# hellosunking/Microcket

Measured on AMD Instinct MI355X. Metric: read-pairs/sec through sam2pairs+dedup (150 bp PE, hg38 names, SAM text resident in HBM), higher is better.
Workload: dtype u8; 1 GPU; C2: 100 M 150 bp PE Micro-C read pairs, hg38, one MI355X -- 100000000 synthetic 150 bp PE read pairs per GPU, hg38 chromosome names, 1 lane(s), unc mode, sam=no, seed 20260105, one step = one pass over the whole resident data set + duplicate marking of the reported pairs on (chr1,pos1,chr2,pos2,strands) + per-chromosome-pair counts; preset=C2, pairs_per_gpu=100000001, sam_bytes_per_gpu=94584442002, block_groups=2097152, blocks=48, parallelism=shard1: independent read-group shards, no data-path collective

## Files before the change

### microcket_amd/csrc/mkt_capi.cpp

```cpp
#include <hip/hip_runtime.h>
#include <stdarg.h>
#include <stdio.h>
#include <stdlib.h>
#include <string.h>
#include <algorithm>
#include <string>
#include <utility>
#include <chrono>
#include <condition_variable>
#include <deque>
#include <mutex>
#include <thread>
#include <vector>

#include "../../include/mkt.h"
#include "mkt_launch.h"

using namespace mkt;

static const size_t kMaxBlock = ((size_t)1 << 31) - 65536;

static thread_local std::string g_create_error;

struct mkt_ctx {
// ... 84 lines not shown
#define HIPCHK(c, call)                                                                            \
    do {                                                                                           \
        hipError_t e_ = (call);                                                                    \
        if (e_ != hipSuccess) return fail((c), MKT_E_HIP, "%s failed: %s", #call, hipGetErrorString(e_)); \
    } while (0)

extern "C" {

int mkt_abi_version(void) { return MKT_ABI_VERSION; }

const char* mkt_strerror(int code) {
    switch (code) {
    case MKT_OK: return "ok";
    case MKT_E_ARG: return "bad argument";
    case MKT_E_NO_DEVICE: return "no usable HIP device (this library has no CPU path)";
    case MKT_E_HIP: return "HIP runtime error";
    case MKT_E_NOMEM: return "out of memory";
    case MKT_E_CAPACITY: return "a QNAME group does not fit the block buffer";
    case MKT_E_KERNEL: return "kernel reported an internal error";
    case MKT_E_STATE: return "call order violated";
    case MKT_E_IO: return "temporary file error";
    default: return "unknown error";
    }
}
const char* mkt_last_error(const mkt_ctx* ctx) { return ctx ? ctx->err.c_str() : g_create_error.c_str(); }

int mkt_device_count(void) {
    int n = 0;
    if (hipGetDeviceCount(&n) != hipSuccess) return 0;
    return n;
}

static size_t ws_tiles_bytes(uint32_t ntiles) {
    size_t b = (size_t)ntiles * (3 * sizeof(uint64_t) + sizeof(TileLast) + sizeof(uint64_t) + sizeof(uint32_t));
    return (b + 127) & ~(size_t)127;
}
static size_t ws_fixed_bytes() { return kMaxRegions * sizeof(RegionCur) + 256 + 1024 * sizeof(uint64_t); }
static size_t ws_bytes_for(uint32_t ntiles) { return ws_tiles_bytes(ntiles) + ws_fixed_bytes() + sizeof(BlockResult); }
static int sync_all(mkt_ctx* c) {
    if (c->s_in) HIPCHK(c, hipStreamSynchronize(c->s_in));
    if (c->stream) HIPCHK(c, hipStreamSynchronize(c->stream));
    if (c->s_out) HIPCHK(c, hipStreamSynchronize(c->s_out));
    return MKT_OK;
}
static int ensure_ws(mkt_ctx* c, uint32_t ntiles) {
    size_t need = ws_bytes_for(ntiles);
    if (need <= c->ws_cap) return MKT_OK;
    need += need / 4;
    if (c->d_ws) { int rc = sync_all(c); if (rc) return rc; HIPCHK(c, hipFree(c->d_ws)); }
    c->d_ws = nullptr; c->ws_cap = 0;
    HIPCHK(c, hipMalloc((void**)&c->d_ws, need));
    c->ws_cap = need;
    return MKT_OK;
}
static int ensure_dev(mkt_ctx* c, uint8_t** p, size_t* cap, size_t need) {
    if (need <= *cap) return MKT_OK;
    if (*p) { int rc = sync_all(c); if (rc) return rc; HIPCHK(c, hipFree(*p)); }
    *p = nullptr; *cap = 0;
    need += need / 8 + 4096;
    HIPCHK(c, hipMalloc((void**)p, need));
    *cap = need;
    return MKT_OK;
}

int mkt_create(const mkt_params* p, mkt_ctx** out) {
    if (!p || !out) return fail(nullptr, MKT_E_ARG, "null argument");
    *out = nullptr;
    if (p->mode != MKT_MODE_FLASH && p->mode != MKT_MODE_UNC) return fail(nullptr, MKT_E_ARG, "mode must be MKT_MODE_FLASH or MKT_MODE_UNC");
    if (p->ref_threads < 2) return fail(nullptr, MKT_E_ARG, "ref_threads must be >= 2 (sam2pairs.cpp:36)");
    int ndev = 0;
// ... 119 lines not shown
    if (!c->d_probe) {
        if (hipMalloc((void**)&c->d_probe, sizeof(unsigned long long)) != hipSuccess) return 0;
        if (hipHostMalloc((void**)&c->h_probe, sizeof(unsigned long long), hipHostMallocDefault) != hipSuccess) return 0;
    }
    if (hipMemsetAsync(c->d_probe, 0, sizeof(unsigned long long), c->stream) != hipSuccess) return 0;
    if (launch_count_newlines(d_text, look, c->d_probe, c->stream) != hipSuccess) return 0;
    if (hipMemcpyAsync(c->h_probe, c->d_probe, sizeof(unsigned long long), hipMemcpyDeviceToHost, c->stream) != hipSuccess) return 0;
    if (hipStreamSynchronize(c->stream) != hipSuccess) return 0;
    return *c->h_probe ? (double)look / (double)*c->h_probe : (double)look;
}
static void smaller_geometry(mkt_ctx* c, const uint8_t* d_text, size_t n) {
    if (c->cfg != CFG_SMALL && d_text) {
        const double avg = probe_device_lines(c, d_text, n);
        const TileDims d = avg > 0 ? lean_dims(avg) : c->dims;
        if (d.tile < c->dims.tile) { c->dims = d; return; }
    }
    if (!shrink_dims(c)) { c->cfg = CFG_SMALL; c->dims = small_dims(); }
}

struct StreamOut { uint8_t* gp; size_t gp_cap; uint8_t* gs; size_t gs_cap; hipEvent_t k0, k1, done; };
static int enqueue_block(mkt_ctx* c, const uint8_t* d_text, size_t n, int cfg, const TileDims& dims, size_t slot, const StreamOut* so = nullptr) {
    if (((uintptr_t)d_text & 15u) != 0) return fail(c, MKT_E_ARG, "block text must be 16-byte aligned");
    if (n >= kMaxBlock) return fail(c, MKT_E_ARG, "block of %zu bytes: must be < 2 GiB - 64 KiB", n);
    const uint32_t ntiles = num_tiles((uint32_t)n, dims.tile);
    int rc = ensure_ws(c, ntiles);
    if (rc) return rc;
    if ((rc = ensure_dev(c, &c->d_pairs, &c->pairs_cap, n / 3 + 65536))) return rc;
    if (c->P.write_sam && (rc = ensure_dev(c, &c->d_sam, &c->sam_cap, n + n / 4 + 65536))) return rc;
    if (!c->d_sc && (rc = ensure_sc_list(c, 1))) return rc;
    KArgs a;
    memset(&a, 0, sizeof a);
    uint8_t* w = c->d_ws;
    a.text = d_text; a.n = (uint32_t)n; a.ntiles = ntiles; a.dims = dims; a.P = c->P;
    a.descA = (uint64_t*)w; w += (size_t)ntiles * 8;
    a.descB = (uint64_t*)w; w += (size_t)ntiles * 8;
    a.descC = (uint64_t*)w; w += (size_t)ntiles * 8;
    a.tile_last = (TileLast*)w; w += (size_t)ntiles * sizeof(TileLast);
    a.tile_groups = (uint64_t*)w; w += (size_t)ntiles * sizeof(uint64_t);
    a.defer_list = (uint32_t*)w;
    w = c->d_ws + ws_tiles_bytes(ntiles);
    a.cur = (RegionCur*)w; w += kMaxRegions * sizeof(RegionCur);
    a.ticket = (uint32_t*)w;
    a.defer_count = (uint32_t*)(w + 64);
    uint32_t* ticket2 = (uint32_t*)(w + 128);
    a.last_tile = (int*)(w + 192);
    a.scan_ticket = (uint32_t*)(w + 224);
    w += 256;
    a.scan_desc = (uint64_t*)w; w += 1024 * sizeof(uint64_t);
    if ((ntiles + finish_chunk_tiles() - 1) / finish_chunk_tiles() > 1024) return fail(c, MKT_E_ARG, "block has too many tiles for the finish scan");
    a.res = (BlockResult*)w;
    a.ordered = c->p.ordered ? 1 : 0;
    a.run = c->d_run;
    a.nregions = c->p.ordered ? 1 : kMaxRegions;
    {
        const size_t need = (size_t)a.nregions * ((n / 256 / (size_t)a.nregions) * 2 + 1024);
        if (c->sc_tmp_cap < need) {
            if (c->d_sc_tmp) { if ((rc = sync_all(c))) return rc; HIPCHK(c, hipFree(c->d_sc_tmp)); }
            c->d_sc_tmp = nullptr; c->sc_tmp_cap = 0;
            HIPCHK(c, hipMalloc((void**)&c->d_sc_tmp, need * sizeof(uint64_t)));
            c->sc_tmp_cap = need;
        }
    }
    a.pairs_rcap = (c->pairs_cap / a.nregions) & ~(uint64_t)15;
    a.sam_rcap = c->P.write_sam ? ((c->sam_cap / a.nregions) & ~(uint64_t)15) : 0;
    a.sc_rcap = c->sc_tmp_cap / a.nregions;
    a.out.pairs = c->d_pairs; a.out.pairs_cap = c->pairs_cap;
    a.out.sam = c->d_sam; a.out.sam_cap = c->P.write_sam ? c->sam_cap : 0;
    a.out.sc = c->d_sc_tmp; a.out.sc_cap = c->sc_tmp_cap;
    a.sc_list = c->d_sc; a.sc_list_cap = c->sc_cap;
    if (c->p.extensions & MKT_EXT_KEYS) {
        if (!c->d_chr) { HIPCHK(c, hipMalloc((void**)&c->d_chr, sizeof(ChrTab))); HIPCHK(c, hipMemsetAsync(c->d_chr, 0, sizeof(ChrTab), c->stream)); }
        const size_t per = (n / 64 / (size_t)a.nregions) * 2 + 4096, need = per * a.nregions;
        if (c->keys_raw_cap < need) {
            if (c->d_keys_raw) { if ((rc = sync_all(c))) return rc; HIPCHK(c, hipFree(c->d_keys_raw)); }
            c->d_keys_raw = nullptr; c->keys_raw_cap = 0;
            HIPCHK(c, hipMalloc((void**)&c->d_keys_raw, need * sizeof(KeyRec)));
            c->keys_raw_cap = need;
        }
        const double per_byte = c->key_density > 0 ? (c->key_density * 2 < 1.0 / 64 ? c->key_density * 2 : 1.0 / 64) : 1.0 / 64;
        const size_t want = (size_t)c->acc.emitted + (size_t)((double)(c->bytes_unsynced + n) * per_byte) + 65536;
        if (c->key_list_cap < want) {
            size_t ncap = c->key_list_cap ? c->key_list_cap * 2 : ((size_t)1 << 22);
            while (ncap < want) ncap *= 2;
            KeyRec* nl = nullptr;
            HIPCHK(c, hipStreamSynchronize(c->stream));
            HIPCHK(c, hipMalloc((void**)&nl, ncap * sizeof(KeyRec)));
            if (c->d_key_list) { HIPCHK(c, hipMemcpy(nl, c->d_key_list, c->key_list_cap * sizeof(KeyRec), hipMemcpyDeviceToDevice)); HIPCHK(c, hipFree(c->d_key_list)); }
            c->d_key_list = nl; c->key_list_cap = ncap;
        }
        a.keys_rcap = c->keys_raw_cap / a.nregions;
        a.out.keys = c->d_keys_raw; a.out.keys_cap = c->keys_raw_cap; a.out.chr = c->d_chr;
        a.out.key_lanes = (c->p.extensions & MKT_EXT_LANES) ? 1u : 0u;
        a.key_list = c->d_key_list; a.key_list_cap = c->key_list_cap;
    }
#if defined(MKT_STAMPS)
    if (!c->d_stamps) { HIPCHK(c, hipMalloc((void**)&c->d_stamps, 16 * sizeof(unsigned long long))); HIPCHK(c, hipMemset(c->d_stamps, 0, 16 * sizeof(unsigned long long))); }
    a.stamps = getenv("MKT_NO_STAMPS") ? nullptr : c->d_stamps;
    { const char* e = getenv("MKT_DEBUG_STOP"); a.debug_stop = e ? atoi(e) : 0; }
#endif
    HIPCHK(c, hipMemsetAsync(c->d_ws, 0, ws_bytes_for(ntiles), c->stream));
    hipEvent_t e0, e1;
    if (so) { e0 = so->k0; e1 = so->k1; }
    else {
        HIPCHK(c, hipEventCreate(&e0));
        HIPCHK(c, hipEventCreate(&e1));
        c->ev.push_back(e0); c->ev.push_back(e1); c->ev_bytes.push_back(n);
    }
    const uint32_t max_wgs = fast_max_workgroups(cfg);
    int grid = (int)(ntiles < max_wgs ? ntiles : max_wgs);
    const bool lean = !c->p.ordered && cfg != CFG_SMALL && !c->no_lean;
    HIPCHK(c, hipEventRecord(e0, c->stream));
    if (lean) {
        HIPCHK(c, launch_fast(a, cfg, grid, c->stream));
        HIPCHK(c, hipEventRecord(e1, c->stream));
        KArgs b = a;
        b.use_list = 1; b.ticket = ticket2;
        HIPCHK(c, launch_tiles(b, cfg, ntiles < 96u ? (int)ntiles : 96, c->stream));
    } else {
        HIPCHK(c, launch_tiles(a, cfg, grid, c->stream));
        HIPCHK(c, hipEventRecord(e1, c->stream));
    }
    HIPCHK(c, launch_finish(a, c->stream));
    if (so) {
        const uint64_t prc = a.nregions > 1 ? a.pairs_rcap : 0, src_ = a.nregions > 1 ? a.sam_rcap : 0;
        HIPCHK(c, launch_gather(a.res, c->d_pairs, prc, so->gp, so->gp_cap, 0, n / 8, c->stream));
        if (c->P.write_sam) HIPCHK(c, launch_gather(a.res, c->d_sam, src_, so->gs, so->gs_cap, 1, n, c->stream));
    }
    HIPCHK(c, hipMemcpyAsync(&c->h_res[slot], a.res, sizeof(BlockResult), hipMemcpyDeviceToHost, c->stream));
    if (so) HIPCHK(c, hipEventRecord(so->done, c->stream));
    return MKT_OK;
}

static void fold_timing(mkt_ctx* c) {
    for (size_t k = 0; k + 1 < c->ev.size(); k += 2) {
        float ms = 0;
        if (hipEventElapsedTime(&ms, c->ev[k], c->ev[k + 1]) == hipSuccess) { c->folded_ms += ms; ++c->folded_launches; c->folded_bytes += c->ev_bytes[k / 2]; }
        (void)hipEventDestroy(c->ev[k]); (void)hipEventDestroy(c->ev[k + 1]);
    }
    c->ev.clear(); c->ev_bytes.clear();
}

static int ensure_sc_list(mkt_ctx* c, size_t need) {
    if (need <= c->sc_cap) return MKT_OK;
    size_t ncap = c->sc_cap ? c->sc_cap : ((size_t)1 << 20);
    while (ncap < need) ncap *= 2;
    uint64_t* nl = nullptr;
    HIPCHK(c, hipMalloc((void**)&nl, ncap * sizeof(uint64_t)));
    if (c->d_sc) {
        if (c->acc.sc) HIPCHK(c, hipMemcpy(nl, c->d_sc, (size_t)c->acc.sc * sizeof(uint64_t), hipMemcpyDeviceToDevice));
        HIPCHK(c, hipFree(c->d_sc));
    }
    c->d_sc = nl; c->sc_cap = ncap;
    return MKT_OK;
}
static void note_sc_density(mkt_ctx* c) {
// ... 1065 lines not shown
```

### microcket_amd/csrc/mkt_kernels.hip

```cpp
#include <hip/hip_runtime.h>
#include <type_traits>
#include "mkt_launch.h"

namespace mkt {

constexpr int NT = 256;
constexpr uint64_t FLAG_AGG = 1ull << 62, FLAG_PREFIX = 2ull << 62, PAYLOAD = (1ull << 62) - 1;
constexpr uint32_t LOOKBACK_SPIN_LIMIT = 1u << 22;

struct ScanScratch { uint64_t a[NT / 64], b[NT / 64]; };

#if defined(MKT_STAMPS)
#define STAMP_DECL() unsigned long long stamp_prev_ = 0, stamp_acc_[16] = {0, 0, 0, 0, 0, 0, 0, 0, 0, 0, 0, 0, 0, 0, 0, 0}
#define STAMP(k)                                                                        \
    do {                                                                                \
        if (tid == 0 && a.stamps) {                                                     \
            const unsigned long long now_ = __builtin_amdgcn_s_memtime();               \
            if ((k) > 0) stamp_acc_[(k)] += now_ - stamp_prev_;                         \
            stamp_prev_ = now_;                                                         \
        }                                                                               \
    } while (0)
#define STAMP_FLUSH(t0_)                                                                \
    do {                                                                                \
        if ((t0_) == 0 && a.stamps) for (int k_ = 1; k_ < 16; ++k_) if (stamp_acc_[k_]) atomicAdd(&a.stamps[k_], stamp_acc_[k_]); \
// ... 134 lines not shown
        uint64_t c = lane <= first ? (w & PAYLOAD) : 0;
#pragma unroll
        for (int d = 32; d >= 1; d >>= 1) c += shfl_xor64(c, d);
        excl += c;
        if (first < 64) break;
        j -= 64;
    }
    if (lane == 0) __hip_atomic_store(&desc[t], FLAG_PREFIX | ((excl + agg) & PAYLOAD), __ATOMIC_RELAXED, __HIP_MEMORY_SCOPE_AGENT);
    return excl;
}

__device__ inline uint32_t claim_ranges(const KArgs& a, uint32_t region, const TileSums& sums, TileSums& base,
                                        uint32_t& region_pair0, uint32_t& region_sam0, OutPtrs& lim) {
    RegionCur* cur = a.cur + region;
    uint32_t err = 0;
    const uint64_t p0 = (uint64_t)region * a.pairs_rcap, s0 = (uint64_t)region * a.sam_rcap, c0 = (uint64_t)region * a.sc_rcap;
    unsigned long long oa = 0, ob = 0;
    if (sums.pair_bytes | sums.emitted) oa = atomicAdd(&cur->a, (unsigned long long)sums.pair_bytes | ((unsigned long long)sums.emitted << kCurShift));
    if (sums.sam_bytes | sums.sc) ob = atomicAdd(&cur->b, (unsigned long long)sums.sam_bytes | ((unsigned long long)sums.sc << kCurShift));
    const uint64_t op = oa & kCurLow, os = ob & kCurLow, oc = ob >> kCurShift;
    if (op + sums.pair_bytes > a.pairs_rcap) err |= E_PAIRS_CAP;
    if (os + sums.sam_bytes > a.sam_rcap) err |= E_SAM_CAP;
    if (oc + sums.sc > a.sc_rcap) err |= E_SC_CAP;
    base.pair_bytes = (uint32_t)(p0 + op); base.sam_bytes = s0 + os; base.sc = (uint32_t)(c0 + oc);
    base.emitted = (uint32_t)((uint64_t)region * a.keys_rcap + (oa >> kCurShift));
    lim.keys_cap = a.keys_rcap ? ((uint64_t)region * a.keys_rcap + ((oa >> kCurShift) + sums.emitted <= a.keys_rcap ? a.keys_rcap : 0)) : 0;
    region_pair0 = (uint32_t)p0; region_sam0 = (uint32_t)s0;
    lim.pairs_cap = err & E_PAIRS_CAP ? 0 : p0 + a.pairs_rcap;
    lim.sam_cap = err & E_SAM_CAP ? 0 : s0 + a.sam_rcap;
    lim.sc_cap = err & E_SC_CAP ? 0 : c0 + a.sc_rcap;
    return err;
}

template <class Cfg>
__global__ __launch_bounds__(NT) void k_tiles(KArgs a) {
    __shared__ TileState<Cfg> st;
    __shared__ ScanScratch scan;
    __shared__ uint32_t s_tile;
    constexpr int NVEC = (Cfg::W + 15) / 16;
    constexpr int NM16 = Cfg::MW * 4;
    constexpr int VPT = (NVEC + NT - 1) / NT;
    constexpr int IPT = (Cfg::LCAP + NT - 1) / NT;
    const int tid = threadIdx.x;
    const Params P = a.P;
    const uint32_t n = a.n;
    __shared__ OutPtrs s_out;
    const uint32_t region = a.nregions > 1 ? (blockIdx.x & (uint32_t)(a.nregions - 1)) : 0u;
    uint16_t* nlmask = reinterpret_cast<uint16_t*>(st.u.m.nlm);
    uint16_t* wsmask = reinterpret_cast<uint16_t*>(st.u.m.wsm);
    STAMP_DECL();

    for (;;) {
        if (tid == 0) {
            s_out = a.out;
            uint32_t k = atomicAdd(a.ticket, 1u);
            if (a.use_list) k = k < *a.defer_count ? a.defer_list[k] : 0xFFFFFFFFu;
            s_tile = k;
            tile_reset(st);
        }
        __syncthreads();
        const uint32_t t = s_tile;
        if (t >= a.ntiles) break;
        STAMP(0);
        const TileGeom G = tile_geom(t, n, a.dims);
        const uint32_t wlen = G.w1 - G.w0;
        const uint32_t nvec = (wlen + 15u) >> 4;
        const TextView tv = tile_view(st, a.text, n, G);

        constexpr int SPT = (NM16 + NT - 1) / NT;
        uint4 xs[SPT];
#pragma unroll
        for (int q = 0; q < SPT; ++q) {
            const uint32_t v = (uint32_t)tid + (uint32_t)q * NT;
            const uint32_t go = G.w0 + (v << 4);
            xs[q] = *reinterpret_cast<const uint4*>(a.text + ((v < nvec && go + 16u <= n) ? go : 0u));
        }
#pragma unroll
        for (int q = 0; q < SPT; ++q) {
            const uint32_t v = (uint32_t)tid + (uint32_t)q * NT;
            if (v >= (uint32_t)NM16) continue;
            uint32_t mnl = 0, mws = 0;
            if (v < nvec) {
                const uint32_t go = G.w0 + (v << 4);
                uint4 x;
                if (go + 16u <= n) {
// ... 120 lines not shown
            if (e) lds_or(&st.err, e);
        }
        if (tid == 5) a.tile_groups[t] = (uint64_t)st.sums.groups | ((uint64_t)st.sums.emitted << 32);
        __syncthreads();
        STAMP(7);

        for (uint32_t i = first_idx + tid; i < end_idx; i += NT) {
            ph_account(st, tv, P, s_out, t, i);
            ph_last(st, &a.tile_last[t], i);
        }
        {
            const uint32_t total = st.sums.pair_bytes;
            const uint64_t go = st.base.pair_bytes;
            if (go + total <= s_out.pairs_cap) { for (uint32_t e = tid; e < st.sums.emitted; e += NT) tile_emit_line(st, tv, e, s_out.pairs + go); }
            else if (tid == 0 && total) lds_or(&st.err, E_PAIRS_CAP);
        }
        if (P.write_sam) {
            for (uint32_t i = first_idx; i < end_idx; ++i) {
                const uint32_t info = st.u.g.g_info[i];
                if ((info & (GI_EMIT | GI_CONTIG)) != (GI_EMIT | GI_CONTIG)) continue;
                const uint32_t len = st.u.g.g_slen[i], src = st.off[i];
                const uint64_t go = st.base.sam_bytes + st.u.g.x_sam[i];
                if (go + len <= s_out.sam_cap) { for (uint32_t k = tid; k < len; k += NT) s_out.sam[go + k] = tv.at(src + k); }
                else if (tid == 0) lds_or(&st.err, E_SAM_CAP);
            }
        }
        __syncthreads();
        STAMP(8);
        if (tid < (int)C_COUNT && st.cnt[tid]) atomicAdd(&a.res->counters[tid], st.cnt[tid]);
        if (tid == 0 && st.err) atomicOr(&a.res->err, st.err);
        __syncthreads();
    }
    STAMP_FLUSH(tid);
}

constexpr int kLoadBatch = 14;
__device__ inline uint32_t nl_xad(uint32_t y, uint32_t nl, uint32_t m1) {
    uint32_t r;
    asm("v_xad_u32 %0, %1, %2, %3" : "=v"(r) : "v"(y), "s"(nl), "v"(m1));
    return r;
}
struct NlConst { uint32_t nl, m1; };
__device__ inline NlConst nl_const() {
    NlConst c;
    c.nl = 0x0A0A0A0Au; c.m1 = 0xFEFEFEFFu;
    asm volatile("" : "+s"(c.nl));
    asm volatile("" : "+v"(c.m1));
    return c;
}
__device__ inline uint64_t has_newline_ballot(const uint4& y, bool valid, const NlConst& c) {
    const uint32_t nl = c.nl, m1 = c.m1;
    const uint32_t r0 = __builtin_amdgcn_bitop3_b32(nl_xad(y.x, nl, m1), y.x, nl, 0x90), r1 = __builtin_amdgcn_bitop3_b32(nl_xad(y.y, nl, m1), y.y, nl, 0x90);
    const uint32_t r2 = __builtin_amdgcn_bitop3_b32(nl_xad(y.z, nl, m1), y.z, nl, 0x90), r3 = __builtin_amdgcn_bitop3_b32(nl_xad(y.w, nl, m1), y.w, nl, 0x90);
    const uint32_t z = __builtin_amdgcn_bitop3_b32(__builtin_amdgcn_bitop3_b32(r0, r1, r2, 0xFE), r3, 0x80808080u, 0xA8);
    return __ballot(z != 0u && valid);
}
template <class Cfg, uint32_t nws>
__device__ inline void fast_scan(const KArgs& a, uint32_t tt, uint64_t* hit, uint32_t ws_, uint32_t kb, uint32_t ke, int lane) {
    const uint32_t ws = (uint32_t)__builtin_amdgcn_readfirstlane((int)ws_);
    const NlConst nlc = nl_const();
    const uint32_t n = a.n;
    const TileGeom G = tile_geom(tt, n, a.dims);
    const uint32_t wlen = G.w1 - G.w0, nvec = (wlen + 15u) >> 4;
    const uint8_t* wbase = a.text + G.w0;
    const uint32_t loff = (uint32_t)lane << 4;
    const uint32_t ngr = nvec >> 6;
// ... 235 lines not shown
                    if ((info & GI_START) && (info & GI_COUNTER) == C_SELFCIRCLE) cc += 1u << 20;
                    cp = g.g_plen[i];
                }
                if (P.write_sam) cs = fast_line_sam(st, G, i);
            }
            uint32_t ec = cc, ep = cp, es = cs, tc, tp, ts;
            block_exscan3<NTW / 64>(ec, ep, es, tc, tp, ts, scan);
            if (tid == 0) {
                st.sums.groups = tc & 0x3FFu; st.sums.emitted = (tc >> 10) & 0x3FFu; st.sums.sc = (tc >> 20) & 0x3FFu;
                st.sums.pair_bytes = tp; st.sums.sam_bytes = ts;
                if (tp > 0xFFFFu) st.abn = AB_PAIR_BYTES;
                else if (!st.abn) {
                    const uint32_t e = claim_ranges(a, region, st.sums, st.base, st.region_pair0, st.region_sam0, s_out);
                    st.region_id = region;
                    if (e) lds_or(&st.abn, e << 8);
                    a.tile_groups[t] = (uint64_t)st.sums.groups | ((uint64_t)st.sums.emitted << 32);
                }
            }
            if (i < NLe && !(st.abn & 0xFFu)) {
                g.x_sam[i] = es;
                if (i < end_idx) {
                    g.x_grp[i] = (uint8_t)(ec & 0xFFu); g.x_sc[i] = (uint8_t)((ec >> 20) & 0xFFu); g.x_emit[i] = (uint8_t)((ec >> 10) & 0xFFu);
                    g.x_pair[i] = (uint16_t)(ep & 0xFFFFu);
                    if (info & GI_EMIT) g.em_idx[(ec >> 10) & 0xFFu] = (uint8_t)i;
                }
            }
        }
        __syncthreads();
        STAMP(6);
        STOP_AFTER(6)
        if (st.abn & 0xFFu) {
            if (tid == 0) {
                a.defer_list[atomicAdd(a.defer_count, 1u)] = t;
                const uint32_t why = st.abn & 0xFFu;
                if (why == AB_NO_PREV || why == AB_OPEN_GROUP) atomicAdd(a.defer_count + 1, 1u);
            }
#if defined(MKT_STAMPS)
            if (tid == 0 && a.stamps) { const uint32_t r = (st.abn & 0xFFu) - 1u; if (r < 12u) atomicAdd(&a.stamps[12 + r / 4u], 1ull << (16u * (r & 3u))); }
#endif
            __syncthreads();
            continue;
        }
        STAMP(7);
        STOP_AFTER(7)

        const uint32_t total = st.sums.pair_bytes;
        uint8_t* const dst = s_out.pairs + st.base.pair_bytes;
        for (uint32_t i = first_idx + ltid; i < end_idx; i += NTW) {
            fast_account(st, s_out, t, i);
            fast_last(st, G, &a.tile_last[t], i);
        }
        if (total && st.base.pair_bytes + total <= s_out.pairs_cap) {
            const auto& g = st.u.g;
            for (uint32_t e = (ltid + (uint32_t)(NTW / 2)) & (uint32_t)(NTW - 1); e < st.sums.emitted; e += NTW) {
                const uint32_t i = g.em_idx[e];
                fast_emit_line(st, g.g_slot[i], g.g_plen[i], dst + g.x_pair[i]);
            }
        }
        __syncthreads();
        STAMP(11);
        if (tid < (int)C_COUNT) wg_cnt[tid] += st.cnt[tid];
        if (tid == 0 && (st.abn >> 8)) atomicOr(&a.res->err, st.abn >> 8);
        const bool sam_copy = P.write_sam && st.sums.sam_bytes && st.base.sam_bytes + st.sums.sam_bytes <= s_out.sam_cap;
        uint32_t* eo = st.rc.f.pos;
        uint32_t* es = st.rc.f.rclip;
        uint32_t E = 0;
// ... 34 lines not shown
                    uint4 xa, xb;
                    __builtin_memcpy(&xa, tbase + so, 16);
                    __builtin_memcpy(&xb, tbase + es[k + 1u] - left, 16);
                    const uint32_t* pa = reinterpret_cast<const uint32_t*>(&xa);
                    const uint32_t* pb = reinterpret_cast<const uint32_t*>(&xb);
                    uint32_t* px = reinterpret_cast<uint32_t*>(&x);
#pragma unroll
                    for (uint32_t q = 0; q < 4u; ++q) {
                        const uint32_t m = left >= 4u * q + 4u ? 0xFFFFFFFFu : (left <= 4u * q ? 0u : (1u << (8u * (left - 4u * q))) - 1u);
                        px[q] = (pa[q] & m) | (pb[q] & ~m);
                    }
                } else {
                    uint32_t q0 = 0, q1 = 0, q2 = 0, q3 = 0;
                    uint32_t kk = k, oo = so, lim = left;
#pragma unroll
                    for (uint32_t b2 = 0; b2 < 16u; ++b2) {
                        while (lim == 0u) { ++kk; oo = es[kk]; lim = eo[kk + 1u] - eo[kk]; }
                        const uint32_t by = (uint32_t)tbase[oo++] << (8u * (b2 & 3u));
                        if (b2 < 4u) q0 |= by; else if (b2 < 8u) q1 |= by; else if (b2 < 12u) q2 |= by; else q3 |= by;
                        --lim;
                    }
                    x = make_uint4(q0, q1, q2, q3);
                }
                *MKT_GLOBAL(uint4, dbase + d) = x;
            }
        }
        __syncthreads();
        STAMP(8);
    }
    if (tid0 < (int)C_COUNT && wg_cnt[tid0]) atomicAdd(&a.res->counters[tid0], wg_cnt[tid0]);
    STAMP_FLUSH(tid0);
}

constexpr int NTF = 1024;
__global__ __launch_bounds__(NTF) void k_finish_scan(KArgs a) {
    __shared__ uint64_t s_wave[NTF / 64];
    __shared__ uint64_t s_pre;
    __shared__ uint32_t s_chunk;
    const int tid = threadIdx.x, lane = tid & 63, wv = tid >> 6;
    if (tid == 0) s_chunk = atomicAdd(a.scan_ticket, 1u);
    __syncthreads();
    const uint32_t chunk = s_chunk;
    const uint32_t t = chunk * NTF + tid;
    const uint64_t x = t < a.ntiles ? a.tile_groups[t] : 0ull;
    if (t < a.ntiles && a.tile_last[t].valid) atomicMax(a.last_tile, (int)t + 1);
    uint64_t inc = x;
#pragma unroll
    for (int d = 1; d < 64; d <<= 1) { uint64_t y = shfl_up64(inc, d); if (lane >= d) inc += y; }
    if (lane == 63) s_wave[wv] = inc;
    __syncthreads();
    uint64_t pre = 0, tot = 0;
    for (int w = 0; w < NTF / 64; ++w) { if (w < wv) pre += s_wave[w]; tot += s_wave[w]; }
    if (wv == 0) {
        const uint64_t ex = lookback(a.scan_desc, chunk, ((tot & 0x7FFFFFFFull) << 31) | (tot >> 32), &a.res->err);
        if (lane == 0) s_pre = (ex >> 31) | ((ex & 0x7FFFFFFFull) << 32);
    }
    __syncthreads();
    if (t < a.ntiles) a.tile_groups[t] = s_pre + pre + inc - x;
    if (chunk == gridDim.x - 1 && tid == 0) a.res->groups = (s_pre + tot) & 0xFFFFFFFFull;
}

constexpr int kFinishGrid = 16;
__global__ __launch_bounds__(NTF) void k_finish(KArgs a) {
    const int tid = threadIdx.x;
    BlockResult* r = a.res;
    __shared__ uint64_t s_scpre[kMaxRegions + 1], s_ca[kMaxRegions], s_cb[kMaxRegions];
    __shared__ uint32_t s_err;
    if (tid < a.nregions) { s_ca[tid] = a.cur[tid].a; s_cb[tid] = a.cur[tid].b; }
    __syncthreads();
    if (tid == 0) {
        uint64_t pb = 0, em = 0, sb = 0, sc = 0;
        uint32_t err = 0;
        for (int q = 0; q < a.nregions; ++q) {
            const uint64_t ca = s_ca[q], cb = s_cb[q];
            const uint64_t p = ca & kCurLow, e = ca >> kCurShift, sm = cb & kCurLow, c = cb >> kCurShift;
            if (blockIdx.x == 0) { r->rpair[q] = p; r->rsam[q] = sm; }
            s_scpre[q] = sc;
            pb += p; em += e; sb += sm; sc += c;
            if (!a.ordered) {
                if (p > a.pairs_rcap) err |= E_PAIRS_CAP;
                if (sm > a.sam_rcap) err |= E_SAM_CAP;
                if (c > a.sc_rcap) err |= E_SC_CAP;
            }
        }
        s_scpre[a.nregions] = sc;
        if (a.ordered) { if (pb > a.out.pairs_cap) err |= E_PAIRS_CAP; if (sb > a.out.sam_cap) err |= E_SAM_CAP; if (sc > a.out.sc_cap) err |= E_SC_CAP; }
        if (a.run->sc + sc > a.sc_list_cap) err |= E_SC_CAP;
        if (a.keys_rcap && a.run->emitted + em > a.key_list_cap) err |= E_SC_CAP;
        s_err = err | r->err;
        if (blockIdx.x == 0) {
            r->pair_bytes = pb; r->emitted = em; r->sam_bytes = sb; r->sc = sc; r->nregions = (uint32_t)a.nregions;
            r->pad = a.defer_count ? *a.defer_count : 0u;
            r->pad2 = a.defer_count ? a.defer_count[1] : 0u;
            r->tiles = a.ntiles;
            const int last = *a.last_tile - 1;
            if (last >= 0) r->last = a.tile_last[last];
        }
    }
    __syncthreads();
    if (s_err == 0) {
        const uint64_t sc_base = a.run->sc, g_base = a.run->groups;
        const int nr = a.nregions;
        const int parts = (int)gridDim.x >= nr ? (int)gridDim.x / nr : 1;
        for (int q = (int)blockIdx.x % nr; q < nr; q += (int)gridDim.x) {
            const int part = (int)blockIdx.x / nr;
            if (part >= parts) break;
            const uint64_t cnt = s_scpre[q + 1] - s_scpre[q];
            const uint64_t* src = a.out.sc + (uint64_t)q * (a.ordered ? 0 : a.sc_rcap);
            for (uint64_t k = (uint64_t)part * NTF + tid; k < cnt; k += (uint64_t)parts * NTF) {
                const uint64_t e = src[k];
                a.sc_list[sc_base + s_scpre[q] + k] = g_base + (a.tile_groups[(uint32_t)(e >> 32)] & 0xFFFFFFFFull) + (uint32_t)(e & 0xFFFFFFFFu);
            }
        }
    }
    __syncthreads();
    if (blockIdx.x == 0 && tid == 0 && (s_err & ~r->err)) r->err |= s_err;
}

__global__ __launch_bounds__(256) void k_keys_place(KArgs a) {
    const BlockResult* r = a.res;
    if (r->err) return;
    __shared__ uint64_t pre[kMaxRegions + 1];
    if (threadIdx.x == 0) {
        uint64_t acc = 0;
        for (int q = 0; q < kMaxRegions; ++q) { pre[q] = acc; if (q < a.nregions) acc += a.cur[q].a >> kCurShift; }
        pre[kMaxRegions] = acc;
    }
    __syncthreads();
    const uint64_t base = a.run->emitted, total = pre[kMaxRegions];
    const uint64_t rstride = a.ordered ? 0 : a.keys_rcap;
    for (uint64_t x = (uint64_t)blockIdx.x * blockDim.x + threadIdx.x; x < total; x += (uint64_t)gridDim.x * blockDim.x) {
        uint32_t q = 0;
#pragma unroll
        for (uint32_t k = 1; k < (uint32_t)kMaxRegions; ++k) q += (x >= pre[k]) ? 1u : 0u;
        KeyRec rec = a.out.keys[(uint64_t)q * rstride + (x - pre[q])];
        const uint64_t ord = base + (a.tile_groups[(uint32_t)(rec.ord >> 16)] >> 32) + (rec.ord & 0xFFFFu);
        rec.ord = ord;
        a.key_list[ord] = rec;
    }
}
__global__ void k_run_advance(KArgs a) {
    BlockResult* r = a.res;
    if (threadIdx.x == 0 && r->err == 0) { a.run->groups += r->groups; a.run->sc += r->sc; a.run->emitted += r->emitted; }
}

struct GatherArgs {
    const BlockResult* res;
    const uint8_t* src; uint64_t rcap;
    uint8_t* dst; uint64_t dst_cap;
    int32_t which;
};
__global__ __launch_bounds__(256) void k_gather(GatherArgs g) {
    __shared__ uint64_t pre[kMaxRegions + 1];
    __shared__ uint64_t s_hole, s_tp;
    const BlockResult* r = g.res;
    if (r->err) return;
    if (threadIdx.x == 0) {
        const uint32_t nr = r->nregions ? r->nregions : 1u;
        uint64_t acc = 0;
        for (uint32_t q = 0; q < (uint32_t)kMaxRegions; ++q) { pre[q] = acc; if (q < nr) acc += g.which ? r->rsam[q] : r->rpair[q]; }
        pre[kMaxRegions] = acc;
        uint64_t tp = 0, hole = acc;
        if (r->last.valid) {
            tp = g.which ? r->last.sam_bytes : r->last.pair_bytes;
            const uint32_t lr = r->last.region < nr ? r->last.region : 0u;
            hole = pre[lr] + (g.which ? r->last.sam_off : r->last.pair_off);
        }
        s_hole = hole; s_tp = tp;
    }
    __syncthreads();
    const uint64_t total = pre[kMaxRegions], tp = s_tp, hole = s_hole, body = total - tp;
    if (total > g.dst_cap) return;
    auto src_of = [&](uint64_t x) -> const uint8_t* {
        const uint64_t y = x < body ? (x < hole ? x : x + tp) : hole + (x - body);
        uint32_t q = 0;
#pragma unroll
// ... 52 lines not shown
    return d.tile >= 16u && !((d.tile | d.hb | d.hf) & 15u) && d.tile <= mx.tile && d.hb <= mx.hb && d.hf <= mx.hf;
}

uint32_t fast_max_workgroups(int) { return 256u * 4u; }

hipError_t launch_tiles(const KArgs& a, int cfg, int grid, hipStream_t s) {
    if (a.ntiles == 0) return hipSuccess;
    if (!dims_ok(a.dims, cfg == CFG_SMALL ? small_dims() : max_dims())) return hipErrorInvalidValue;
    if (cfg == CFG_SMALL) hipLaunchKernelGGL(k_tiles<CfgSmall>, dim3(grid), dim3(NT), 0, s, a);
    else hipLaunchKernelGGL(k_tiles<CfgFast>, dim3(grid), dim3(NT), 0, s, a);
    return hipGetLastError();
}
hipError_t launch_fast(const KArgs& a, int, int grid, hipStream_t s) {
    if (a.ntiles == 0) return hipSuccess;
    if (!dims_ok(a.dims, max_dims())) return hipErrorInvalidValue;
    hipLaunchKernelGGL((k_fast<CfgLean, NT, 2, 4>), dim3(grid), dim3(NT), 0, s, a);
    return hipGetLastError();
}
__global__ void k_count_nl(const uint8_t* text, size_t n, unsigned long long* out) {
    unsigned long long mine = 0;
    const size_t nv = n >> 4;
    for (size_t v = (size_t)blockIdx.x * blockDim.x + threadIdx.x; v < nv; v += (size_t)gridDim.x * blockDim.x) {
        const uint4 x = reinterpret_cast<const uint4*>(text)[v];
        mine += __popc(nl_flags(x.x)) + __popc(nl_flags(x.y)) + __popc(nl_flags(x.z)) + __popc(nl_flags(x.w));
    }
    if (blockIdx.x == 0 && threadIdx.x == 0) for (size_t b = nv << 4; b < n; ++b) mine += text[b] == '\n';
    for (int d = 32; d >= 1; d >>= 1) mine += shfl_xor64(mine, d);
    if ((threadIdx.x & 63) == 0 && mine) atomicAdd(out, mine);
}
hipError_t launch_count_newlines(const uint8_t* text, size_t n, unsigned long long* out, hipStream_t s) {
    if (n) hipLaunchKernelGGL(k_count_nl, dim3(64), dim3(256), 0, s, text, n, out);
    return hipGetLastError();
}
hipError_t launch_finish(const KArgs& a, hipStream_t s) {
    const unsigned chunks = (a.ntiles + NTF - 1) / NTF;
    if (chunks) hipLaunchKernelGGL(k_finish_scan, dim3(chunks), dim3(NTF), 0, s, a);
    hipLaunchKernelGGL(k_finish, dim3(kFinishGrid), dim3(NTF), 0, s, a);
    if (a.keys_rcap) hipLaunchKernelGGL(k_keys_place, dim3(2048), dim3(256), 0, s, a);
    hipLaunchKernelGGL(k_run_advance, dim3(1), dim3(64), 0, s, a);
    return hipGetLastError();
}
uint32_t finish_chunk_tiles() { return NTF; }

constexpr int DD_WG = 256;
constexpr int DS_WG = 512;
constexpr int DS_NW = DS_WG / 64;
constexpr int DS_T = 8192;
constexpr int DS_K = DS_T / DS_WG;
constexpr int DS_D = 7, DS_R = 1 << DS_D;
constexpr int DS_SCAN_WG = 1024, DS_SCAN_V = 8;
constexpr uint64_t kKeyMask1 = 0xFFFFFFFFC000FFFFull;
static_assert(DS_R == 2 * 64, "the scatter's prologue gives each lane of wave 0 two digits");

__device__ inline bool key_eq(const KeyRec& x, const KeyRec& y) { return x.k0 == y.k0 && (x.k1 & kKeyMask1) == (y.k1 & kKeyMask1); }

__global__ __launch_bounds__(DS_WG) void k_dd_prep(const KeyRec* keys, uint64_t n, int ib, uint64_t* rec, uint32_t* cnt, uint32_t G) {
    __shared__ uint32_t c[DS_R];
    if (threadIdx.x < DS_R) c[threadIdx.x] = 0;
    __syncthreads();
    const uint64_t b = (uint64_t)blockIdx.x * DS_T, e = b + DS_T < n ? b + DS_T : n, hi = ~((1ull << ib) - 1ull);
    for (uint64_t j = b + threadIdx.x; j < e; j += DS_WG) {
        const uint64_t r = (mix64(keys[j].k0 ^ mix64(keys[j].k1 & kKeyMask1)) & hi) | j;
        rec[j] = r;
        atomicAdd(&c[(r >> ib) & (DS_R - 1)], 1u);
    }
    __syncthreads();
    if (threadIdx.x < DS_R) cnt[threadIdx.x * G + blockIdx.x] = c[threadIdx.x];
}
__global__ __launch_bounds__(DS_WG) void k_dd_count(const uint64_t* rec, uint64_t n, int shift, uint32_t* cnt, uint32_t G) {
    __shared__ uint32_t c[DS_R];
    if (threadIdx.x < DS_R) c[threadIdx.x] = 0;
    __syncthreads();
    const uint64_t b = (uint64_t)blockIdx.x * DS_T, m = (b + DS_T < n ? b + DS_T : n) - b;
    const ulonglong2* v = reinterpret_cast<const ulonglong2*>(rec + b);
    for (uint64_t i = threadIdx.x; i < m / 2; i += DS_WG) {
// ... 382 lines not shown
```

### microcket_amd/csrc/mkt_launch.h

```cpp
#pragma once
#include <hip/hip_runtime.h>
#include "mkt_host.h"
#include "mkt_fast.h"
#include "mkt_synth.h"

namespace mkt {

enum { CFG_FAST = 0, CFG_SMALL = 1 };

struct DevRun { uint64_t groups, sc, emitted; };

struct alignas(128) RegionCur { unsigned long long a, b; unsigned long long pad[14]; };
constexpr int kMaxRegions = 16;
constexpr int kCurShift = 36;
constexpr unsigned long long kCurLow = (1ull << kCurShift) - 1ull;

struct KArgs {
    const uint8_t* text;
    uint32_t n;
    uint32_t ntiles;
    TileDims dims;
    Params P;
    uint64_t* descA;
    uint64_t* descB;
    uint64_t* descC;
    uint32_t* ticket;
    uint64_t* tile_groups;
    int32_t ordered;
    TileLast* tile_last;
    uint32_t* defer_list;
    uint32_t* defer_count;
    int* last_tile;
    uint64_t* scan_desc;
    uint32_t* scan_ticket;
    int32_t use_list;
    BlockResult* res;
    DevRun* run;
    RegionCur* cur;
    int32_t nregions;
    uint64_t pairs_rcap, sam_rcap, sc_rcap;
    uint64_t* sc_list;
    uint64_t sc_list_cap;
    uint64_t keys_rcap;
    KeyRec* key_list;
    uint64_t key_list_cap;
    OutPtrs out;
    unsigned long long* stamps;
    int32_t debug_stop;
};

TileDims small_dims();
TileDims max_dims();
uint32_t fast_max_workgroups(int cfg);
hipError_t launch_count_newlines(const uint8_t* text, size_t n, unsigned long long* out, hipStream_t s);
hipError_t launch_tiles(const KArgs& a, int cfg, int grid, hipStream_t s);
hipError_t launch_fast(const KArgs& a, int cfg, int grid, hipStream_t s);
uint32_t finish_chunk_tiles();
hipError_t launch_finish(const KArgs& a, hipStream_t s);
hipError_t launch_gather(const BlockResult* d_res, const uint8_t* src, uint64_t rcap, uint8_t* dst, uint64_t dst_cap, int which, uint64_t max_bytes, hipStream_t s);
hipError_t launch_sc_logged(const uint64_t* list, uint64_t n, uint64_t drop_group, uint64_t group_offset, uint64_t K_total, uint32_t ref_threads,
                            unsigned long long* out, hipStream_t s);

struct DedupResult { uint64_t total, dups; };
hipError_t launch_dedup(const KeyRec* keys, uint64_t n, uint8_t* flags, void* work, size_t work_bytes, DedupResult* d_res, hipStream_t s);
size_t dedup_work_bytes(uint64_t n);
size_t radix64_count_bytes(uint64_t n);
hipError_t launch_radix64(uint64_t*& rA, uint64_t*& rB, uint64_t n, int lo_bit, int nbits, uint32_t* cnt, hipStream_t s);
size_t partition_work_bytes();
hipError_t launch_partition(const KeyRec* keys, uint64_t n, const uint16_t* d_lut, uint32_t world, uint32_t* hist, KeyRec* send, uint32_t* perm, uint32_t* G_out, hipStream_t s);
hipError_t launch_unpermute(const uint8_t* in, const uint32_t* perm, uint64_t n, uint8_t* out, unsigned long long* dups, hipStream_t s);
hipError_t launch_chrstat(const KeyRec* keys, uint64_t n, const uint16_t* dense_of_slot, uint32_t ndense, unsigned long long* counts, hipStream_t s);

hipError_t launch_synth_sizes(const SynParams& p, uint64_t first, uint64_t n, uint64_t* sizes, hipStream_t s);
hipError_t launch_exscan(uint64_t* v, uint64_t n, uint64_t* total, hipStream_t s);
hipError_t launch_synth_write(const SynParams& p, uint64_t first, uint64_t n, const uint64_t* offs, char* out, hipStream_t s);
hipError_t launch_synth_tail(const SynParams& p, char* out, hipStream_t s);
size_t synth_tail_bytes(const SynParams& p);

}
```

Baseline: 2.081 billion read-pairs/s.

## Fold tile-group scan into last tile workgroup and merge finish kernels

The separate finish-scan, finish, keys-place and run-advance kernels are replaced: the last workgroup of k_tiles (detected with a completion counter) performs the tile_groups prefix scan with vectorized loads, and a single epilogue kernel does the sc-list and key-list placement plus the run-counter advance in its last workgroup. The per-tile workspace memset is skipped on the lean path, with the fast kernel writing zeros for deferred tiles instead. This removes several kernel launches and a full workspace clear per block. In exchange, the scan now runs serially in one workgroup, and correctness depends on every tile slot being written before the scan.

```diff
diff --git a/microcket_amd/csrc/mkt_capi.cpp b/microcket_amd/csrc/mkt_capi.cpp
--- a/microcket_amd/csrc/mkt_capi.cpp
+++ b/microcket_amd/csrc/mkt_capi.cpp
@@ -140,10 +140,10 @@
 }
 
 static size_t ws_tiles_bytes(uint32_t ntiles) {
-    size_t b = (size_t)ntiles * (3 * sizeof(uint64_t) + sizeof(TileLast) + sizeof(uint64_t) + sizeof(uint32_t));
+    size_t b = (((size_t)ntiles + 1) & ~(size_t)1) * sizeof(uint64_t) + (size_t)ntiles * (3 * sizeof(uint64_t) + sizeof(TileLast) + sizeof(uint32_t));
     return (b + 127) & ~(size_t)127;
 }
-static size_t ws_fixed_bytes() { return kMaxRegions * sizeof(RegionCur) + 256 + 1024 * sizeof(uint64_t); }
+static size_t ws_fixed_bytes() { return kMaxRegions * sizeof(RegionCur) + 256; }
 static size_t ws_bytes_for(uint32_t ntiles) { return ws_tiles_bytes(ntiles) + ws_fixed_bytes() + sizeof(BlockResult); }
 static int sync_all(mkt_ctx* c) {
     if (c->s_in) HIPCHK(c, hipStreamSynchronize(c->s_in));
@@ -329,11 +329,11 @@
     memset(&a, 0, sizeof a);
     uint8_t* w = c->d_ws;
     a.text = d_text; a.n = (uint32_t)n; a.ntiles = ntiles; a.dims = dims; a.P = c->P;
+    a.tile_groups = (uint64_t*)w; w += (((size_t)ntiles + 1) & ~(size_t)1) * sizeof(uint64_t);
     a.descA = (uint64_t*)w; w += (size_t)ntiles * 8;
     a.descB = (uint64_t*)w; w += (size_t)ntiles * 8;
     a.descC = (uint64_t*)w; w += (size_t)ntiles * 8;
     a.tile_last = (TileLast*)w; w += (size_t)ntiles * sizeof(TileLast);
-    a.tile_groups = (uint64_t*)w; w += (size_t)ntiles * sizeof(uint64_t);
     a.defer_list = (uint32_t*)w;
     w = c->d_ws + ws_tiles_bytes(ntiles);
     a.cur = (RegionCur*)w; w += kMaxRegions * sizeof(RegionCur);
@@ -341,10 +341,9 @@
     a.defer_count = (uint32_t*)(w + 64);
     uint32_t* ticket2 = (uint32_t*)(w + 128);
     a.last_tile = (int*)(w + 192);
-    a.scan_ticket = (uint32_t*)(w + 224);
+    a.tiles_done = (uint32_t*)(w + 224);
+    a.epi_done = (uint32_t*)(w + 240);
     w += 256;
-    a.scan_desc = (uint64_t*)w; w += 1024 * sizeof(uint64_t);
-    if ((ntiles + finish_chunk_tiles() - 1) / finish_chunk_tiles() > 1024) return fail(c, MKT_E_ARG, "block has too many tiles for the finish scan");
     a.res = (BlockResult*)w;
     a.ordered = c->p.ordered ? 1 : 0;
     a.run = c->d_run;
@@ -395,7 +394,14 @@
     a.stamps = getenv("MKT_NO_STAMPS") ? nullptr : c->d_stamps;
     { const char* e = getenv("MKT_DEBUG_STOP"); a.debug_stop = e ? atoi(e) : 0; }
 #endif
-    HIPCHK(c, hipMemsetAsync(c->d_ws, 0, ws_bytes_for(ntiles), c->stream));
+    const bool lean = !c->p.ordered && cfg != CFG_SMALL && !c->no_lean;
+#if defined(MKT_STAMPS)
+    const bool fill_all = true;
+#else
+    const bool fill_all = !lean;
+#endif
+    if (fill_all) HIPCHK(c, hipMemsetAsync(c->d_ws, 0, ws_bytes_for(ntiles), c->stream));
+    else HIPCHK(c, hipMemsetAsync(c->d_ws + ws_tiles_bytes(ntiles), 0, ws_fixed_bytes() + sizeof(BlockResult), c->stream));
     hipEvent_t e0, e1;
     if (so) { e0 = so->k0; e1 = so->k1; }
     else {
@@ -405,7 +411,6 @@
     }
     const uint32_t max_wgs = fast_max_workgroups(cfg);
     int grid = (int)(ntiles < max_wgs ? ntiles : max_wgs);
-    const bool lean = !c->p.ordered && cfg != CFG_SMALL && !c->no_lean;
     HIPCHK(c, hipEventRecord(e0, c->stream));
     if (lean) {
         HIPCHK(c, launch_fast(a, cfg, grid, c->stream));
@@ -417,7 +422,7 @@
         HIPCHK(c, launch_tiles(a, cfg, grid, c->stream));
         HIPCHK(c, hipEventRecord(e1, c->stream));
     }
-    HIPCHK(c, launch_finish(a, c->stream));
+    HIPCHK(c, launch_epilogue(a, c->stream));
     if (so) {
         const uint64_t prc = a.nregions > 1 ? a.pairs_rcap : 0, src_ = a.nregions > 1 ? a.sam_rcap : 0;
         HIPCHK(c, launch_gather(a.res, c->d_pairs, prc, so->gp, so->gp_cap, 0, n / 8, c->stream));
diff --git a/microcket_amd/csrc/mkt_kernels.hip b/microcket_amd/csrc/mkt_kernels.hip
--- a/microcket_amd/csrc/mkt_kernels.hip
+++ b/microcket_amd/csrc/mkt_kernels.hip
@@ -190,6 +190,74 @@
     return err;
 }
 
+__device__ inline bool arrive_last(uint32_t* done, uint32_t* s_flag) {
+    asm volatile("s_waitcnt vmcnt(0) lgkmcnt(0)" ::: "memory");
+    __syncthreads();
+    if (threadIdx.x == 0) {
+        __builtin_amdgcn_fence(__ATOMIC_RELEASE, "agent");
+        asm volatile("s_waitcnt vmcnt(0)" ::: "memory");
+        const uint32_t last = __hip_atomic_fetch_add(done, 1u, __ATOMIC_RELAXED, __HIP_MEMORY_SCOPE_AGENT) == gridDim.x - 1u ? 1u : 0u;
+        if (last) { __builtin_amdgcn_fence(__ATOMIC_ACQUIRE, "agent"); asm volatile("s_waitcnt vmcnt(0)" ::: "memory"); }
+        *s_flag = last;
+    }
+    __syncthreads();
+    return *s_flag != 0u;
+}
+
+__device__ inline void scan_tile_groups(const KArgs& a, ScanScratch& sc) {
+    constexpr uint32_t NW = NT / 64, U = 4;
+    const uint32_t lane = threadIdx.x & 63u, wv = threadIdx.x >> 6;
+    const uint32_t nv = (a.ntiles + 1u) >> 1;
+    const uint32_t per = ((nv + NW * 64u - 1u) / (NW * 64u)) * 64u;
+    const uint32_t v0 = wv * per < nv ? wv * per : nv, v1 = v0 + per < nv ? v0 + per : nv;
+    uint4* const vec = reinterpret_cast<uint4*>(a.tile_groups);
+    auto load = [&](uint32_t v, uint64_t& x, uint64_t& y) {
+        x = 0; y = 0;
+        if (v < v1) {
+            const uint4 q = vec[v];
+            x = (uint64_t)q.x | ((uint64_t)q.y << 32);
+            if (2u * v + 1u < a.ntiles) y = (uint64_t)q.z | ((uint64_t)q.w << 32);
+        }
+    };
+    uint64_t sum = 0;
+    uint32_t last = 0;
+    for (uint32_t vb = v0; vb < v1; vb += 64u * U) {
+        uint64_t x[U], y[U];
+#pragma unroll
+        for (uint32_t k = 0; k < U; ++k) load(vb + 64u * k + lane, x[k], y[k]);
+#pragma unroll
+        for (uint32_t k = 0; k < U; ++k) {
+            const uint32_t v = vb + 64u * k + lane;
+            sum += x[k] + y[k];
+            if ((uint32_t)y[k]) last = 2u * v + 2u; else if ((uint32_t)x[k]) last = 2u * v + 1u;
+        }
+    }
+#pragma unroll
+    for (int d = 32; d >= 1; d >>= 1) { sum += shfl_xor64(sum, d); const uint32_t o = (uint32_t)__shfl_xor((int)last, d, 64); last = o > last ? o : last; }
+    if (lane == 0) { sc.a[wv] = sum; sc.b[wv] = last; }
+    __syncthreads();
+    uint64_t carry = 0, total = 0;
+    uint32_t last_all = 0;
+    for (uint32_t w = 0; w < NW; ++w) { if (w < wv) carry += sc.a[w]; total += sc.a[w]; last_all = (uint32_t)sc.b[w] > last_all ? (uint32_t)sc.b[w] : last_all; }
+    for (uint32_t vb = v0; vb < v1; vb += 64u * U) {
+        uint64_t x[U], y[U];
+#pragma unroll
+        for (uint32_t k = 0; k < U; ++k) load(vb + 64u * k + lane, x[k], y[k]);
+#pragma unroll
+        for (uint32_t k = 0; k < U; ++k) {
+            const uint32_t v = vb + 64u * k + lane;
+            const uint64_t s = x[k] + y[k];
+            uint64_t inc = s;
+#pragma unroll
+            for (int d = 1; d < 64; d <<= 1) { const uint64_t o = shfl_up64(inc, d); if ((int)lane >= d) inc += o; }
+            const uint64_t ex = carry + inc - s, ey = ex + x[k];
+            if (v < v1) vec[v] = make_uint4((uint32_t)ex, (uint32_t)(ex >> 32), (uint32_t)ey, (uint32_t)(ey >> 32));
+            carry += (uint64_t)__shfl((long long)inc, 63, 64);
+        }
+    }
+    if (threadIdx.x == 0) { a.res->groups = total & 0xFFFFFFFFull; *a.last_tile = (int)last_all; }
+}
+
 template <class Cfg>
 __global__ __launch_bounds__(NT) void k_tiles(KArgs a) {
     __shared__ TileState<Cfg> st;
@@ -208,7 +276,8 @@
     uint16_t* wsmask = reinterpret_cast<uint16_t*>(st.u.m.wsm);
     STAMP_DECL();
 
-    for (;;) {
+    const bool idle = a.use_list && *a.defer_count == 0u;
+    if (!idle) for (;;) {
         if (tid == 0) {
             s_out = a.out;
             uint32_t k = atomicAdd(a.ticket, 1u);
@@ -395,6 +464,7 @@
         __syncthreads();
     }
     STAMP_FLUSH(tid);
+    if (arrive_last(a.tiles_done, &s_tile)) scan_tile_groups(a, scan);
 }
 
 constexpr int kLoadBatch = 14;
@@ -696,6 +766,7 @@
         if (st.abn & 0xFFu) {
             if (tid == 0) {
                 a.defer_list[atomicAdd(a.defer_count, 1u)] = t;
+                a.tile_groups[t] = 0;
                 const uint32_t why = st.abn & 0xFFu;
                 if (why == AB_NO_PREV || why == AB_OPEN_GROUP) atomicAdd(a.defer_count + 1, 1u);
             }
@@ -796,50 +867,25 @@
     STAMP_FLUSH(tid0);
 }
 
-constexpr int NTF = 1024;
-__global__ __launch_bounds__(NTF) void k_finish_scan(KArgs a) {
-    __shared__ uint64_t s_wave[NTF / 64];
-    __shared__ uint64_t s_pre;
-    __shared__ uint32_t s_chunk;
-    const int tid = threadIdx.x, lane = tid & 63, wv = tid >> 6;
-    if (tid == 0) s_chunk = atomicAdd(a.scan_ticket, 1u);
-    __syncthreads();
-    const uint32_t chunk = s_chunk;
-    const uint32_t t = chunk * NTF + tid;
-    const uint64_t x = t < a.ntiles ? a.tile_groups[t] : 0ull;
-    if (t < a.ntiles && a.tile_last[t].valid) atomicMax(a.last_tile, (int)t + 1);
-    uint64_t inc = x;
-#pragma unroll
-    for (int d = 1; d < 64; d <<= 1) { uint64_t y = shfl_up64(inc, d); if (lane >= d) inc += y; }
-    if (lane == 63) s_wave[wv] = inc;
-    __syncthreads();
-    uint64_t pre = 0, tot = 0;
-    for (int w = 0; w < NTF / 64; ++w) { if (w < wv) pre += s_wave[w]; tot += s_wave[w]; }
-    if (wv == 0) {
-        const uint64_t ex = lookback(a.scan_desc, chunk, ((tot & 0x7FFFFFFFull) << 31) | (tot >> 32), &a.res->err);
-        if (lane == 0) s_pre = (ex >> 31) | ((ex & 0x7FFFFFFFull) << 32);
-    }
-    __syncthreads();
-    if (t < a.ntiles) a.tile_groups[t] = s_pre + pre + inc - x;
-    if (chunk == gridDim.x - 1 && tid == 0) a.res->groups = (s_pre + tot) & 0xFFFFFFFFull;
-}
-
-constexpr int kFinishGrid = 16;
-__global__ __launch_bounds__(NTF) void k_finish(KArgs a) {
+constexpr int kEpilogueWG = 256;
+__global__ __launch_bounds__(kEpilogueWG) void k_epilogue(KArgs a) {
+    __shared__ uint64_t s_scpre[kMaxRegions + 1], s_kpre[kMaxRegions + 1], s_ca[kMaxRegions], s_cb[kMaxRegions];
+    __shared__ uint32_t s_err, s_flag;
     const int tid = threadIdx.x;
     BlockResult* r = a.res;
-    __shared__ uint64_t s_scpre[kMaxRegions + 1], s_ca[kMaxRegions], s_cb[kMaxRegions];
-    __shared__ uint32_t s_err;
+    const uint64_t g_base = a.run->groups, sc_base = a.run->sc, em_base = a.run->emitted, blk_groups = r->groups;
+    const uint32_t err_in = r->err;
     if (tid < a.nregions) { s_ca[tid] = a.cur[tid].a; s_cb[tid] = a.cur[tid].b; }
     __syncthreads();
     if (tid == 0) {
         uint64_t pb = 0, em = 0, sb = 0, sc = 0;
         uint32_t err = 0;
-        for (int q = 0; q < a.nregions; ++q) {
+        for (int q = 0; q < kMaxRegions; ++q) {
+            s_scpre[q] = sc; s_kpre[q] = em;
+            if (q >= a.nregions) continue;
             const uint64_t ca = s_ca[q], cb = s_cb[q];
             const uint64_t p = ca & kCurLow, e = ca >> kCurShift, sm = cb & kCurLow, c = cb >> kCurShift;
             if (blockIdx.x == 0) { r->rpair[q] = p; r->rsam[q] = sm; }
-            s_scpre[q] = sc;
             pb += p; em += e; sb += sm; sc += c;
             if (!a.ordered) {
                 if (p > a.pairs_rcap) err |= E_PAIRS_CAP;
@@ -847,65 +893,48 @@
                 if (c > a.sc_rcap) err |= E_SC_CAP;
             }
         }
-        s_scpre[a.nregions] = sc;
+        s_scpre[kMaxRegions] = sc; s_kpre[kMaxRegions] = em;
         if (a.ordered) { if (pb > a.out.pairs_cap) err |= E_PAIRS_CAP; if (sb > a.out.sam_cap) err |= E_SAM_CAP; if (sc > a.out.sc_cap) err |= E_SC_CAP; }
-        if (a.run->sc + sc > a.sc_list_cap) err |= E_SC_CAP;
-        if (a.keys_rcap && a.run->emitted + em > a.key_list_cap) err |= E_SC_CAP;
-        s_err = err | r->err;
+        if (sc_base + sc > a.sc_list_cap) err |= E_SC_CAP;
+        if (a.keys_rcap && em_base + em > a.key_list_cap) err |= E_SC_CAP;
+        s_err = err | err_in;
         if (blockIdx.x == 0) {
             r->pair_bytes = pb; r->emitted = em; r->sam_bytes = sb; r->sc = sc; r->nregions = (uint32_t)a.nregions;
-            r->pad = a.defer_count ? *a.defer_count : 0u;
-            r->pad2 = a.defer_count ? a.defer_count[1] : 0u;
+            r->pad = a.defer_count[0];
+            r->pad2 = a.defer_count[1];
             r->tiles = a.ntiles;
             const int last = *a.last_tile - 1;
             if (last >= 0) r->last = a.tile_last[last];
-        }
-    }
-    __syncthreads();
-    if (s_err == 0) {
-        const uint64_t sc_base = a.run->sc, g_base = a.run->groups;
-        const int nr = a.nregions;
-        const int parts = (int)gridDim.x >= nr ? (int)gridDim.x / nr : 1;
-        for (int q = (int)blockIdx.x % nr; q < nr; q += (int)gridDim.x) {
-            const int part = (int)blockIdx.x / nr;
-            if (part >= parts) break;
-            const uint64_t cnt = s_scpre[q + 1] - s_scpre[q];
-            const uint64_t* src = a.out.sc + (uint64_t)q * (a.ordered ? 0 : a.sc_rcap);
-            for (uint64_t k = (uint64_t)part * NTF + tid; k < cnt; k += (uint64_t)parts * NTF) {
-                const uint64_t e = src[k];
-                a.sc_list[sc_base + s_scpre[q] + k] = g_base + (a.tile_groups[(uint32_t)(e >> 32)] & 0xFFFFFFFFull) + (uint32_t)(e & 0xFFFFFFFFu);
-            }
-        }
-    }
-    __syncthreads();
-    if (blockIdx.x == 0 && tid == 0 && (s_err & ~r->err)) r->err |= s_err;
-}
-
-__global__ __launch_bounds__(256) void k_keys_place(KArgs a) {
-    const BlockResult* r = a.res;
-    if (r->err) return;
-    __shared__ uint64_t pre[kMaxRegions + 1];
-    if (threadIdx.x == 0) {
-        uint64_t acc = 0;
-        for (int q = 0; q < kMaxRegions; ++q) { pre[q] = acc; if (q < a.nregions) acc += a.cur[q].a >> kCurShift; }
-        pre[kMaxRegions] = acc;
-    }
-    __syncthreads();
-    const uint64_t base = a.run->emitted, total = pre[kMaxRegions];
-    const uint64_t rstride = a.ordered ? 0 : a.keys_rcap;
-    for (uint64_t x = (uint64_t)blockIdx.x * blockDim.x + threadIdx.x; x < total; x += (uint64_t)gridDim.x * blockDim.x) {
-        uint32_t q = 0;
-#pragma unroll
-        for (uint32_t k = 1; k < (uint32_t)kMaxRegions; ++k) q += (x >= pre[k]) ? 1u : 0u;
-        KeyRec rec = a.out.keys[(uint64_t)q * rstride + (x - pre[q])];
-        const uint64_t ord = base + (a.tile_groups[(uint32_t)(rec.ord >> 16)] >> 32) + (rec.ord & 0xFFFFu);
-        rec.ord = ord;
-        a.key_list[ord] = rec;
-    }
-}
-__global__ void k_run_advance(KArgs a) {
-    BlockResult* r = a.res;
-    if (threadIdx.x == 0 && r->err == 0) { a.run->groups += r->groups; a.run->sc += r->sc; a.run->emitted += r->emitted; }
+            if (s_err != err_in) r->err = s_err;
+        }
+    }
+    __syncthreads();
+    const uint32_t err = s_err;
+    if (err == 0) {
+        const uint64_t n_sc = s_scpre[kMaxRegions], n_all = n_sc + (a.keys_rcap ? s_kpre[kMaxRegions] : 0ull);
+        const uint64_t sc_stride = a.ordered ? 0 : a.sc_rcap, key_stride = a.ordered ? 0 : a.keys_rcap;
+        for (uint64_t x = (uint64_t)blockIdx.x * kEpilogueWG + tid; x < n_all; x += (uint64_t)gridDim.x * kEpilogueWG) {
+            const bool is_sc = x < n_sc;
+            const uint64_t y = is_sc ? x : x - n_sc;
+            const uint64_t* pre = is_sc ? s_scpre : s_kpre;
+            uint32_t q = 0;
+#pragma unroll
+            for (uint32_t k = 1; k < (uint32_t)kMaxRegions; ++k) q += (y >= pre[k]) ? 1u : 0u;
+            if (is_sc) {
+                const uint64_t e = a.out.sc[(uint64_t)q * sc_stride + (y - pre[q])];
+                a.sc_list[sc_base + y] = g_base + (a.tile_groups[(uint32_t)(e >> 32)] & 0xFFFFFFFFull) + (uint32_t)(e & 0xFFFFFFFFu);
+            } else {
+                KeyRec rec = a.out.keys[(uint64_t)q * key_stride + (y - pre[q])];
+                const uint64_t ord = em_base + (a.tile_groups[(uint32_t)(rec.ord >> 16)] >> 32) + (rec.ord & 0xFFFFu);
+                rec.ord = ord;
+                if (ord < a.key_list_cap) a.key_list[ord] = rec;
+            }
+        }
+    }
+    if (arrive_last(a.epi_done, &s_flag) && tid == 0 && err == 0) {
+        DevRun* run = a.run;
+        run->groups = g_base + blk_groups; run->sc = sc_base + s_scpre[kMaxRegions]; run->emitted = em_base + s_kpre[kMaxRegions];
+    }
 }
 
 struct GatherArgs {
@@ -1024,15 +1053,12 @@
     if (n) hipLaunchKernelGGL(k_count_nl, dim3(64), dim3(256), 0, s, text, n, out);
     return hipGetLastError();
 }
-hipError_t launch_finish(const KArgs& a, hipStream_t s) {
-    const unsigned chunks = (a.ntiles + NTF - 1) / NTF;
-    if (chunks) hipLaunchKernelGGL(k_finish_scan, dim3(chunks), dim3(NTF), 0, s, a);
-    hipLaunchKernelGGL(k_finish, dim3(kFinishGrid), dim3(NTF), 0, s, a);
-    if (a.keys_rcap) hipLaunchKernelGGL(k_keys_place, dim3(2048), dim3(256), 0, s, a);
-    hipLaunchKernelGGL(k_run_advance, dim3(1), dim3(64), 0, s, a);
+hipError_t launch_epilogue(const KArgs& a, hipStream_t s) {
+    uint64_t grid = a.keys_rcap ? (uint64_t)a.n / 256u / kEpilogueWG + 1u : 16u;
+    grid = grid < 16u ? 16u : (grid > 1024u ? 1024u : grid);
+    hipLaunchKernelGGL(k_epilogue, dim3((unsigned)grid), dim3(kEpilogueWG), 0, s, a);
     return hipGetLastError();
 }
-uint32_t finish_chunk_tiles() { return NTF; }
 
 constexpr int DD_WG = 256;
 constexpr int DS_WG = 512;
diff --git a/microcket_amd/csrc/mkt_launch.h b/microcket_amd/csrc/mkt_launch.h
--- a/microcket_amd/csrc/mkt_launch.h
+++ b/microcket_amd/csrc/mkt_launch.h
@@ -31,8 +31,8 @@
     uint32_t* defer_list;
     uint32_t* defer_count;
     int* last_tile;
-    uint64_t* scan_desc;
-    uint32_t* scan_ticket;
+    uint32_t* tiles_done;
+    uint32_t* epi_done;
     int32_t use_list;
     BlockResult* res;
     DevRun* run;
@@ -55,8 +55,7 @@
 hipError_t launch_count_newlines(const uint8_t* text, size_t n, unsigned long long* out, hipStream_t s);
 hipError_t launch_tiles(const KArgs& a, int cfg, int grid, hipStream_t s);
 hipError_t launch_fast(const KArgs& a, int cfg, int grid, hipStream_t s);
-uint32_t finish_chunk_tiles();
-hipError_t launch_finish(const KArgs& a, hipStream_t s);
+hipError_t launch_epilogue(const KArgs& a, hipStream_t s);
 hipError_t launch_gather(const BlockResult* d_res, const uint8_t* src, uint64_t rcap, uint8_t* dst, uint64_t dst_cap, int which, uint64_t max_bytes, hipStream_t s);
 hipError_t launch_sc_logged(const uint64_t* list, uint64_t n, uint64_t drop_group, uint64_t group_offset, uint64_t K_total, uint32_t ref_threads,
                             unsigned long long* out, hipStream_t s);
```

New measurement: 1.957 billion read-pairs/s. 0.94x the previous value.
